# AzureLeon1/DiffSpectra

Measured on AMD Instinct MI355X. Metric: molecules/sec, 1000-step QM9S all-spectra sampling (partial run), higher is better.
Workload: dtype f32 (GEMMs as split-fp16 x3 MFMA with fp32 accumulate; fp32-level accuracy, parity gates unchanged)

## Files before the change

diffspectra_amd/csrc/ds_forward.hip:

```cpp
#include <hip/hip_runtime.h>
#include <math.h>
#include <stdint.h>
#include <stdlib.h>

#include <atomic>
#include <mutex>
#include <utility>
#include <vector>

#include "../../include/diffspectra_hip.h"
#include "../../include/diffspectra_step.h"
#include "../../include/diffspectra_tiles.h"
#include "ds_device.h"
#include "ds_host.h"

#define ADAC DS_ADA_COLS
constexpr int DS_NODE_PF = 8;
constexpr int DS_NODE_PF2 = 4;
constexpr int DS_QKV_PF = 4;
constexpr int DS_QKV_PF_WIDE = 4;
constexpr int DS_NODE_TILE64_MIN_PER_CU = 4;
constexpr int DS_TWO_STREAM_MAX_PAIRS = 400000;

#ifdef DS_STAMPS
// ... 787 lines not shown
#pragma unroll
        for (int cc = 0; cc < 2; ++cc) {
          const float bf = b1[half * 256 + (wave + 4 * cc) * 32 + (tid & 31)];
#pragma unroll
          for (int i = 0; i < 16; ++i) acc[cc][0][i] = bf;
          acc_zero<1>(lo[cc]);
        }
        wave_mma_h_ring_t2<1, false, 16, DS_NODE_PF2>(&H2[0][0], 256, wstream_h(W1, 512, 256, (half * 8 + wave) * 32),
                                                     wstream_h(W1, 512, 256, (half * 8 + wave + 4) * 32), 0, acc[0], lo[0], acc[1], lo[1]);
#pragma unroll
        for (int cc = 0; cc < 2; ++cc) {
          split_finish<1>(acc[cc], lo[cc]);
          const int colf = (wave + 4 * cc) * 32 + (tid & 31);
#pragma unroll
          for (int i = 0; i < 16; i += 2) {
            f32x2 v;
            v.x = acc[cc][0][i]; v.y = acc[cc][0][i + 1];
            v = ds_silu2(v);
            const int r0 = acc_row(i, hhf);
            split_store1(&B1[r0][0], 256, colf, v.x);
            split_store1(&B1[r0 + 1][0], 256, colf, v.y);
          }
        }
      }
      __syncthreads();
      asm volatile("" ::: "memory");
      wave_mma_h_ring_t2<1, false, 16, DS_NODE_PF2>(&B1[0][0], 256, wstream_h(W2, 256, 512, wave * 32), wstream_h(W2, 256, 512, (wave + 4) * 32),
                                                   half * 16, acc2[0], lo2[0], acc2[1], lo2[1], half * 16);
      __syncthreads();
    }
    split_finish<1>(acc2[0], lo2[0]);
    split_finish<1>(acc2[1], lo2[1]);
    const int hhl = (tid & 63) >> 5;
    const bool two = mB - mA <= 1;
    bool isB[16];
#pragma unroll
    for (int i = 0; i < 16; ++i) isB[i] = rmol[acc_row(i, hhl)] != mA;
    const int rows_here = Nn - row0;
#pragma unroll
    for (int cc = 0; cc < 2; ++cc) {
      const int col = (wave + 4 * cc) * 32 + (tid & 31);
      const float gA = gAv[cc], gB = gBv[cc], bb = bbv[cc];
      const RowStore st = row_store<256>(c.ws.h + (size_t)row0 * 256 + (wave + 4 * cc) * 32);
#pragma unroll
      for (int i = 0; i < 16; ++i) {
        const int row = acc_row(i, hhl);
        float g = isB[i] ? gB : gA;
        if (!two) { const int m = rmol[row]; if (m != mA && m != mB) g = gsec[(size_t)m * ADAC + col]; }
        const float out = split_load1(&H2[row][0], 256, col) + g * (acc2[cc][0][i] + bb);
        split_store1(&H2[row][0], 256, col, out);
        if (row < rows_here) row_put(st, ((i & 3) + 8 * (i >> 2)) * 256 * 4, out);
      }
    }
  }
  __syncthreads();
  {
    const float* br = BW(c, blk, DS_BW_NODE_RO_B);
    auto ws_of = [&](int it) {
      return it < 2 ? wstream_h(BW(c, blk, DS_BW_NODE_RO_H), 64, 256, it * 32) : wstream_h(BW(c, blk, DS_BW_AC_H), 512, 256, (it - 2) * 32);
    };
    auto bias_of = [&](int it) { return it < 2 ? br[it * 32 + (tid & 31)] : 0.0f; };
    auto store_of = [&](int it, const f32x16 (&acc)[1]) {
      if (it < 2) acc_store<1, 768>(acc, c.ws.atom_hids + (size_t)row0 * 768 + 256 + 64 * blk + it * 32, Nn - row0, [](int, float v) { return v; });
      else acc_store<1, 512>(acc, c.ws.ac + (size_t)row0 * 512 + (it - 2) * 32, Nn - row0, [](int, float v) { return v; });
    };
#pragma unroll
    for (int pr = 0; pr < 2; ++pr) {
      asm volatile("" ::: "memory");
      const int itA = wave + 8 * pr, itB = itA + 4;
      f32x16 acc[2][1], lo[2][1];
      const float bA = bias_of(itA), bB = bias_of(itB);
#pragma unroll
      for (int i = 0; i < 16; ++i) { acc[0][0][i] = bA; acc[1][0][i] = bB; }
      acc_zero<1>(lo[0]); acc_zero<1>(lo[1]);
      wave_mma_h_ring_t2<1, false, 16, DS_NODE_PF2>(&H2[0][0], 256, ws_of(itA), ws_of(itB), 0, acc[0], lo[0], acc[1], lo[1]);
      split_finish<1>(acc[0], lo[0]);
      store_of(itA, acc[0]);
      split_finish<1>(acc[1], lo[1]);
      store_of(itB, acc[1]);
    }
    if (wave < 2) {
      asm volatile("" ::: "memory");
      const int it = 16 + wave;
      f32x16 acc[1], lo[1];
      acc_zero<1>(acc);
      acc_zero<1>(lo);
      wave_mma_h_ring<1, false, 16, DS_NODE_PF>(&H2[0][0], 256, BW(c, blk, DS_BW_AC_H), 512, 256, (it - 2) * 32, 0, acc, lo);
      split_finish<1>(acc, lo);
      store_of(it, acc);
    }
  }
}

constexpr int DS_GATE_SLOTS = 16;
template <bool N2E>
__global__ __launch_bounds__(512) void k_node_update64(Ctx c, int blk) {
  ds_fp16_saturate();
  constexpr int T = 64, LDH = 2 * 256 + 8, GS = DS_GATE_SLOTS;
  __shared__ __attribute__((aligned(16))) _Float16 B1[T][LDH];
  __shared__ __attribute__((aligned(16))) _Float16 H2[T][LDH];
  __shared__ __attribute__((aligned(16))) float G[GS][256];
  __shared__ int rmol[T], rslot[T], smol[T], nslot;
  const int tid = threadIdx.x, wave = tid >> 6, row0 = blockIdx.x * T;
  const int Nn = c.L.Nn;
  const float* ada = c.ws.ada;
  const float* gsec = ada + blk * DS_ADA_BLOCK_STRIDE + DS_ADA_NODE + 1280;
  float4 va[2][4], vh[2][4];
#pragma unroll
  for (int ps = 0; ps < 2; ++ps) {
    const size_t gr = (size_t)min(row0 + 8 * wave + 4 * ps + ((tid & 63) >> 4), Nn - 1);
    const float4* ap = reinterpret_cast<const float4*>(c.ws.attn + gr * 256) + (tid & 15);
    const float4* hp = reinterpret_cast<const float4*>(c.ws.h + gr * 256) + (tid & 15);
#pragma unroll
    for (int u = 0; u < 4; ++u) {
      va[ps][u] = ap[16 * u];
      vh[ps][u] = hp[16 * u];
    }
  }
  if (tid < T) {
    const bool in = row0 + tid < Nn;
    const int m = in ? c.L.node_mol[row0 + tid] : 0;
    const bool first = in && (tid == 0 || c.L.node_mol[row0 + tid - 1] != m);
    const unsigned long long starts = __ballot(first);
    const int slot = __popcll(starts & ((2ull << tid) - 1ull)) - 1;
    rmol[tid] = m;
    rslot[tid] = slot;
    if (first) smol[slot] = m;
    if (tid == 0) nslot = __popcll(starts);
  }
  __syncthreads();
  const int ns = nslot;
  {
    const int lane = tid & 63, g = lane >> 4, j = lane & 15;
    float4 vg[2][4], sh[2][4], sc[2][4], gv[2];
#pragma unroll
    for (int ps = 0; ps < 2; ++ps) {
      const int row = 8 * wave + 4 * ps + g;
      const float4* ad = reinterpret_cast<const float4*>(ada + (size_t)rmol[row] * ADAC + blk * DS_ADA_BLOCK_STRIDE + DS_ADA_NODE) + j;
#pragma unroll
      for (int u = 0; u < 4; ++u) {
        vg[ps][u] = ad[128 + 16 * u];
        sh[ps][u] = ad[192 + 16 * u];
        sc[ps][u] = ad[256 + 16 * u];
      }
    }
#pragma unroll
    for (int u = 0; u < 2; ++u)
      gv[u] = reinterpret_cast<const float4*>(gsec + (size_t)smol[min(wave + 8 * u, ns - 1)] * ADAC)[lane];
#pragma unroll
    for (int ps = 0; ps < 2; ++ps) {
      const int row = 8 * wave + 4 * ps + g;
      float4 r[4];
#pragma unroll
      for (int u = 0; u < 4; ++u) {
        if (row0 + row >= Nn) va[ps][u] = vh[ps][u] = make_float4(0, 0, 0, 0);
        if (N2E) split_store4(&B1[row][0], 256, 64 * u + 4 * j, va[ps][u]);
        r[u].x = vh[ps][u].x + vg[ps][u].x * va[ps][u].x; r[u].y = vh[ps][u].y + vg[ps][u].y * va[ps][u].y;
        r[u].z = vh[ps][u].z + vg[ps][u].z * va[ps][u].z; r[u].w = vh[ps][u].w + vg[ps][u].w * va[ps][u].w;
      }
      ln_mod_quad256(r, sh[ps], sc[ps]);
#pragma unroll
      for (int u = 0; u < 4; ++u) split_store4(&H2[row][0], 256, 64 * u + 4 * j, r[u]);
    }
#pragma unroll
    for (int u = 0; u < 2; ++u) reinterpret_cast<float4*>(&G[wave + 8 * u][0])[lane] = gv[u];
  }
  const float* W1 = BW(c, blk, DS_BW_FF1_H);
  const float* W2 = BW(c, blk, DS_BW_FF2_H);
  auto tail_ws = [&](int it) {
    return it < 2 ? wstream_h(BW(c, blk, DS_BW_NODE_RO_H), 64, 256, it * 32) : wstream_h(BW(c, blk, DS_BW_AC_H), 512, 256, (it - 2) * 32);
  };
  WRingH<DS_NODE_PF> ring, ring_n2e;
  const bool n2e = N2E && wave < 4 && row0 + (wave >> 1) * 32 < Nn;
  const WStreamH wsn = wstream_h(BW(c, blk, DS_BW_N2E_H), 64, 256, (wave & 1) * 32);
  if (n2e) wring_h<DS_NODE_PF>(ring_n2e, wsn, 0);
  wring_h<DS_NODE_PF>(ring, wstream_h(W1, 512, 256, wave * 32), 0);
  __syncthreads();
  if (N2E) {
    {
      const int mt = wave >> 1, cc = wave & 1;
      if (n2e) {
        f32x16 acc[1], lo[1];
        acc_zero<1>(acc);
        acc_zero<1>(lo);
        wave_mma_h_deep<1, false, 16, DS_NODE_PF>(&B1[mt * 32][0], 256, wsn, ring_n2e, 0, acc, lo);
        split_finish<1>(acc, lo);
        acc_store<1, 64>(acc, c.ws.u + (size_t)(row0 + mt * 32) * 64 + cc * 32, Nn - row0 - mt * 32, [](int, float v) { return v; });
      }
    }
    __syncthreads();
  }
  {
    const float* b1 = BW(c, blk, DS_BW_FF1_B);
    const WStreamH ws2 = wstream_h(W2, 256, 512, wave * 32);
    f32x16 acc2[2], lo2[2];
    acc_zero<2>(acc2);
    acc_zero<2>(lo2);
    const int col = wave * 32 + (tid & 31);
    const float bb = BW(c, blk, DS_BW_FF2_B)[col];
    for (int half = 0; half < 2; ++half) {
      {
        asm volatile("" ::: "memory");
        const int hhf = (tid & 63) >> 5;
        f32x16 acc[2], lo[2];
        const float bf = b1[half * 256 + col];
#pragma unroll
        for (int m = 0; m < 2; ++m)
#pragma unroll
          for (int i = 0; i < 16; ++i) acc[m][i] = bf;
        acc_zero<2>(lo);
        wave_mma_h_deep<2, false, 16, DS_NODE_PF>(&H2[0][0], 256, wstream_h(W1, 512, 256, (half * 8 + wave) * 32), ring, 0, acc, lo);
        wring_h<DS_NODE_PF>(ring, ws2, half * 16);
        split_finish<2>(acc, lo);
#pragma unroll
        for (int m = 0; m < 2; ++m)
#pragma unroll
          for (int i = 0; i < 16; i += 2) {
            f32x2 v;
            v.x = acc[m][i]; v.y = acc[m][i + 1];
            v = ds_silu2(v);
            const int r0 = m * 32 + acc_row(i, hhf);
            split_store1(&B1[r0][0], 256, col, v.x);
            split_store1(&B1[r0 + 1][0], 256, col, v.y);
          }
      }
      __syncthreads();
      asm volatile("" ::: "memory");
      wave_mma_h_deep<2, false, 16, DS_NODE_PF>(&B1[0][0], 256, ws2, ring, half * 16, acc2, lo2, half * 16);
      wring_h<DS_NODE_PF>(ring, half == 0 ? wstream_h(W1, 512, 256, (8 + wave) * 32) : tail_ws(wave), 0);
      __syncthreads();
    }
    split_finish<2>(acc2, lo2);
    float* Gx = reinterpret_cast<float*>(&B1[0][0]);
    if (ns > GS) {
      for (int idx = tid; idx < (ns - GS) * 64; idx += 512)
        reinterpret_cast<float4*>(Gx)[idx] = reinterpret_cast<const float4*>(gsec + (size_t)smol[GS + (idx >> 6)] * ADAC)[idx & 63];
      __syncthreads();
    }
    const int hhl = (tid & 63) >> 5;
    const int rows_here = Nn - row0;
    const RowStore st = row_store<256>(c.ws.h + (size_t)row0 * 256 + wave * 32);
#pragma unroll
    for (int m = 0; m < 2; ++m)
#pragma unroll
      for (int i = 0; i < 16; ++i) {
        const int row = m * 32 + acc_row(i, hhl), s = rslot[row];
        const float g = s < GS ? G[s][col] : Gx[(s - GS) * 256 + col];
        const float out = split_load1(&H2[row][0], 256, col) + g * (acc2[m][i] + bb);
        split_store1(&H2[row][0], 256, col, out);
        if (row < rows_here) row_put(st, (m * 32 + (i & 3) + 8 * (i >> 2)) * 256 * 4, out);
      }
  }
  __syncthreads();
  {
    const float* br = BW(c, blk, DS_BW_NODE_RO_B);
    const int mt = (wave >> 1) & 1, itl = 16 + (wave & 1);
    const bool last = wave >= 4 && row0 + mt * 32 < Nn;
#pragma unroll
    for (int pr = 0; pr < 2; ++pr) {
      asm volatile("" ::: "memory");
      const int it = wave + 8 * pr;
      const float bi = it < 2 ? br[it * 32 + (tid & 31)] : 0.0f;
      f32x16 acc[2], lo[2];
#pragma unroll
      for (int m = 0; m < 2; ++m)
#pragma unroll
        for (int i = 0; i < 16; ++i) acc[m][i] = bi;
      acc_zero<2>(lo);
      wave_mma_h_deep<2, false, 16, DS_NODE_PF>(&H2[0][0], 256, tail_ws(it), ring, 0, acc, lo);
      if (pr == 0) wring_h<DS_NODE_PF>(ring, tail_ws(wave + 8), 0);
      else if (last) wring_h<DS_NODE_PF>(ring, tail_ws(itl), 0);
      split_finish<2>(acc, lo);
      if (it < 2) acc_store<2, 768>(acc, c.ws.atom_hids + (size_t)row0 * 768 + 256 + 64 * blk + it * 32, Nn - row0, [](int, float v) { return v; });
      else acc_store<2, 512>(acc, c.ws.ac + (size_t)row0 * 512 + (it - 2) * 32, Nn - row0, [](int, float v) { return v; });
    }
    if (last) {
      asm volatile("" ::: "memory");
      f32x16 acc[1], lo[1];
      acc_zero<1>(acc);
      acc_zero<1>(lo);
      wave_mma_h_deep<1, false, 16, DS_NODE_PF>(&H2[mt * 32][0], 256, tail_ws(itl), ring, 0, acc, lo);
      split_finish<1>(acc, lo);
      acc_store<1, 512>(acc, c.ws.ac + (size_t)(row0 + mt * 32) * 512 + (itl - 2) * 32, Nn - row0 - mt * 32, [](int, float v) { return v; });
    }
  }
}

__global__ __launch_bounds__(256, 2) void k_edge_update(Ctx c, int blk) {
  ds_fp16_saturate();
  DS_STAMP_INIT();
  constexpr int R = 32, LDW = 64 + DS_LDP;
  __shared__ __attribute__((aligned(16))) float E2s[4][R][LDW];
  __shared__ __attribute__((aligned(16))) float Ds[4][R][LDW];
  __shared__ int idx_s[4][3][R];
  const int tid = threadIdx.x, wave = tid >> 6, lane = tid & 63, hh = lane >> 5, r31 = lane & 31;
  constexpr int LDW2 = 2 * 64 + 8;
  float(*E2)[LDW] = E2s[wave];
  _Float16* E2h = reinterpret_cast<_Float16*>(&E2s[wave][0][0]);
  _Float16* Dh = reinterpret_cast<_Float16*>(&Ds[wave][0][0]);
  int* rmol = idx_s[wave][0];
  int* rpa = idx_s[wave][1];
  int* rpb = idx_s[wave][2];
  const int Pp = c.L.Pp;
  const int row0 = (blockIdx.x * 4 + wave) * R;
  if (row0 >= Pp) return;
  const int valid = min(R, Pp - row0);
  const float* ada = c.ws.ada + blk * DS_ADA_BLOCK_STRIDE + DS_ADA_EDGE;
  if (lane < R) {
    const int p = min(row0 + lane, Pp - 1);
    rmol[lane] = c.L.pair_mol[p]; rpa[lane] = c.L.pair_a[p]; rpb[lane] = c.L.pair_b[p];
  }
  DS_STAMP(0);
  {
    const float4* bn = reinterpret_cast<const float4*>(BW(c, blk, DS_BW_N2E_B));
    float rm[4], rs[4], ra[4];
#pragma unroll
    for (int t = 0; t < 4; ++t) {
      const int k = 4 * (lane & 15) + t;
      rm[t] = k ? BW(c, blk, DS_BW_RBF_MEAN)[k - 1] : 0.0f;
      rs[t] = __builtin_amdgcn_rcpf(k ? BW(c, blk, DS_BW_RBF_STD)[k - 1] : 1.0f);
      ra[t] = __builtin_amdgcn_rcpf(k ? BW(c, blk, DS_BW_RBF_ASTD)[k - 1] : 1.0f);
    }
#pragma unroll
    for (int it = 0; it < 2; ++it) {
      float4 ua[4], ub[4], ve[4], vd[4], vg[4], sh[4], sc[4];
      float xd[4];
#pragma unroll
      for (int u = 0; u < 4; ++u) {
        const int idx = lane + (it * 4 + u) * 64, row = idx >> 4, k4 = idx & 15;
        const size_t pc = (size_t)min(row0 + row, Pp - 1);
        const float* ad = ada + (size_t)rmol[row] * ADAC;
        ua[u] = reinterpret_cast<const float4*>(c.ws.u + (size_t)rpa[row] * 64)[k4];
        ub[u] = reinterpret_cast<const float4*>(c.ws.u + (size_t)rpb[row] * 64)[k4];
        ve[u] = reinterpret_cast<const float4*>(c.ws.e + pc * 64)[k4];
        xd[u] = c.ws.dist[pc];
        vg[u] = reinterpret_cast<const float4*>(ad + 128)[k4];
        sh[u] = reinterpret_cast<const float4*>(ad + 192)[k4];
        sc[u] = reinterpret_cast<const float4*>(ad + 256)[k4];
      }
#pragma unroll
      for (int u = 0; u < 4; ++u) {
        const int idx = lane + (it * 4 + u) * 64, row = idx >> 4, k4 = idx & 15;
        const float4 b = bn[k4];
        float4 r;
        r.x = ve[u].x + vg[u].x * ((ua[u].x + ub[u].x) + b.x); r.y = ve[u].y + vg[u].y * ((ua[u].y + ub[u].y) + b.y);
        r.z = ve[u].z + vg[u].z * ((ua[u].z + ub[u].z) + b.z); r.w = ve[u].w + vg[u].w * ((ua[u].w + ub[u].w) + b.w);
        r = ln_mod_reg64(r, sh[u], sc[u]);
        {
          float f[4];
#pragma unroll
          for (int t = 0; t < 4; ++t) {
            const float z = (xd[u] - rm[t]) * rs[t];
            f[t] = __expf(-0.5f * (z * z)) * ra[t];
          }
          if (k4 == 0) f[0] = xd[u];
          vd[u] = make_float4(f[0], f[1], f[2], f[3]);
        }
        if (row >= valid) { r = make_float4(0, 0, 0, 0); vd[u] = r; }
        split_store4(E2h + row * LDW2, 64, 4 * k4, r);
        split_store4(Dh + row * LDW2, 64, 4 * k4, vd[u]);
      }
    }
  }
  DS_STAMP(1);
  f32x16 a4[2][1], a4lo[2][1];
  acc_zero<1>(a4[0]); acc_zero<1>(a4[1]);
  acc_zero<1>(a4lo[0]); acc_zero<1>(a4lo[1]);
  {
    const float* b3 = BW(c, blk, DS_BW_FF3_B);
    const float* W3 = BW(c, blk, DS_BW_FF3_H);
    const uint4* W4 = reinterpret_cast<const uint4*>(BW(c, blk, DS_BW_FF4_C)) + lane;
#pragma unroll
    for (int hc = 0; hc < 4; ++hc) {
      f32x16 a3[1], a3lo[1];
#pragma unroll
      for (int q = 0; q < 4; ++q) {
        const float4 bb = *reinterpret_cast<const float4*>(b3 + hc * 32 + 8 * q + 4 * hh);
        a3[0][4 * q] = bb.x; a3[0][4 * q + 1] = bb.y; a3[0][4 * q + 2] = bb.z; a3[0][4 * q + 3] = bb.w;
      }
      acc_zero<1>(a3lo);
      wave_mma_h<1, true, 4>(E2h, 64, W3, 128, 64, hc * 32, 0, 4, a3, a3lo);
      split_finish<1>(a3, a3lo);
#pragma unroll
      for (int s_ = 0; s_ < 2; ++s_) {
        h8 y1, y2;
#pragma unroll
        for (int j = 0; j < 8; j += 2) {
          f32x2 v;
          v.x = a3[0][8 * s_ + j]; v.y = a3[0][8 * s_ + j + 1];
          v = ds_silu2(v);
          y1[j] = (_Float16)v.x; y1[j + 1] = (_Float16)v.y;
          y2[j] = (_Float16)((v.x - (float)y1[j]) * 2048.0f); y2[j + 1] = (_Float16)((v.y - (float)y1[j + 1]) * 2048.0f);
        }
#pragma unroll
        for (int ft = 0; ft < 2; ++ft) {
          const h8 w1 = __builtin_bit_cast(h8, W4[(((0 * 4 + hc) * 2 + s_) * 2 + ft) * 64]);
          const h8 w2 = __builtin_bit_cast(h8, W4[(((1 * 4 + hc) * 2 + s_) * 2 + ft) * 64]);
          a4[ft][0] = __builtin_amdgcn_mfma_f32_32x32x16_f16(w1, y1, a4[ft][0], 0, 0, 0);
          a4lo[ft][0] = __builtin_amdgcn_mfma_f32_32x32x16_f16(w1, y2, a4lo[ft][0], 0, 0, 0);
          a4lo[ft][0] = __builtin_amdgcn_mfma_f32_32x32x16_f16(w2, y1, a4lo[ft][0], 0, 0, 0);
        }
      }
    }
    split_finish<1>(a4[0], a4lo[0]);
    split_finish<1>(a4[1], a4lo[1]);
  }
  DS_STAMP(2);
  {
    const float* b4 = BW(c, blk, DS_BW_FF4_B);
    const float* grow = ada + (size_t)rmol[r31] * ADAC + 320;
    float4 xo[2][4];
#pragma unroll
    for (int ft = 0; ft < 2; ++ft)
#pragma unroll
      for (int q = 0; q < 4; ++q) {
        const int n0 = ft * 32 + 8 * q + 4 * hh;
        const float4 g = *reinterpret_cast<const float4*>(grow + n0);
        const float4 bb = *reinterpret_cast<const float4*>(b4 + n0);
        const h4 p0 = *reinterpret_cast<const h4*>(E2h + r31 * LDW2 + n0);
        const h4 p1 = *reinterpret_cast<const h4*>(E2h + r31 * LDW2 + 64 + n0);
        float4 x;
        x.x = fmaf((float)p1[0], 1.0f / 2048.0f, (float)p0[0]); x.y = fmaf((float)p1[1], 1.0f / 2048.0f, (float)p0[1]);
        x.z = fmaf((float)p1[2], 1.0f / 2048.0f, (float)p0[2]); x.w = fmaf((float)p1[3], 1.0f / 2048.0f, (float)p0[3]);
        x.x += g.x * (a4[ft][0][4 * q + 0] + bb.x); x.y += g.y * (a4[ft][0][4 * q + 1] + bb.y);
        x.z += g.z * (a4[ft][0][4 * q + 2] + bb.z); x.w += g.w * (a4[ft][0][4 * q + 3] + bb.w);
        xo[ft][q] = x;
      }
    __builtin_amdgcn_fence(__ATOMIC_ACQ_REL, "workgroup");
    __builtin_amdgcn_wave_barrier();
#pragma unroll
    for (int ft = 0; ft < 2; ++ft)
#pragma unroll
      for (int q = 0; q < 4; ++q) *reinterpret_cast<float4*>(&E2[r31][ft * 32 + 8 * q + 4 * hh]) = xo[ft][q];
  }
#pragma unroll
  for (int u = 0; u < 8; ++u) {
    const int idx = lane + u * 64, row = idx >> 4, k4 = idx & 15;
    const float4 v = reinterpret_cast<const float4*>(&E2[row][0])[k4];
    if (row < valid) reinterpret_cast<float4*>(c.ws.e + (size_t)(row0 + row) * 64)[k4] = v;
  }
  DS_STAMP(3);
  {
    f32x16 acc[1];
    acc_zero<1>(acc);
    wave_mma<1>(&E2[0][0], LDW, BW(c, blk, DS_BW_EDGE_RO_W), 32, 0, 0, 8, acc);
    if (r31 < 16) {
      const float b = BW(c, blk, DS_BW_EDGE_RO_B)[r31];
      acc_store<1, 192>(acc, c.ws.edge_hids + (size_t)row0 * 192 + 64 + 16 * blk, valid, [b](int, float v) { return v + b; });
    }
  }
  DS_STAMP(4);
  {
    float4 v[8];
#pragma unroll
    for (int u = 0; u < 8; ++u) v[u] = reinterpret_cast<const float4*>(&E2[(lane + u * 64) >> 4][0])[lane & 15];
    __builtin_amdgcn_fence(__ATOMIC_ACQ_REL, "workgroup");
    __builtin_amdgcn_wave_barrier();
#pragma unroll
    for (int u = 0; u < 8; ++u) split_store4(E2h + ((lane + u * 64) >> 4) * LDW2, 64, 4 * (lane & 15), v[u]);
  }
  DS_STAMP(5);
  {
    const float* bd = BW(c, blk, DS_BW_ED_B);
    const float* Wd = BW(c, blk, DS_BW_ED_H);
    float* ed = c.ws.ed + (size_t)row0 * 256;
    for (int ch = 0; ch < 8; ++ch) {
      asm volatile("" ::: "memory");
      f32x16 acc[1], lo[1];
      const float b = bd[ch * 32 + r31];
#pragma unroll
      for (int i = 0; i < 16; ++i) acc[0][i] = b;
      acc_zero<1>(lo);
      wave_mma_h<1>(E2h, 64, Wd, 256, 128, ch * 32, 0, 4, acc, lo);
      wave_mma_h<1>(Dh, 64, Wd, 256, 128, ch * 32, 4, 8, acc, lo, 4);
      split_finish<1>(acc, lo);
      acc_store<1, 256>(acc, ed + ch * 32, valid, [](int, float v) { return v; });
    }
  }
  DS_STAMP(6);
  DS_STAMP_FLUSH(0);
}

constexpr int EQUI_NCW = 4;
constexpr int EQUI_NLW = 4;
__global__ __launch_bounds__((EQUI_NCW + EQUI_NLW) * 64) void k_equi_pairs(Ctx c, int blk) {
  ds_fp16_saturate();
  constexpr int NCW = EQUI_NCW, NLW = EQUI_NLW;
  constexpr int T = 64, TP = 32, LDH = 2 * 256 + 8, NCH = 8;
  constexpr int CPW = NCH / NCW;
  constexpr int PPW = TP / NLW;
  constexpr int NPASS = PPW / 2;
  static_assert(NCH % NCW == 0 && TP % NLW == 0 && PPW % 2 == 0, "role split");
  static_assert(CPW == 2, "a consumer wave runs its two feature chunks against shared X fragments");
  __shared__ __attribute__((aligned(16))) _Float16 Xh[2][T][LDH];
  __shared__ __attribute__((aligned(16))) float part[2][NCH][T][4];
  __shared__ __attribute__((aligned(16))) float dirs[3][T][4];
  __shared__ __attribute__((aligned(16))) float cb0[NCH][2][16];
  __shared__ __attribute__((aligned(16))) float cw2[NCH][2][4][16];
  const int tid = threadIdx.x, wave = tid >> 6, lane = tid & 63, hh = lane >> 5;
  const int Pp = c.L.Pp;
  const int ntiles_all = (Pp + TP - 1) / TP;
  const int tiles_per_wg = (ntiles_all + (int)gridDim.x - 1) / (int)gridDim.x;
  const int ntiles = min(ntiles_all, ((int)blockIdx.x + 1) * tiles_per_wg);
  const float* adq = c.ws.ada + blk * DS_ADA_BLOCK_STRIDE + DS_ADA_EQUI;
  const bool consumer = wave < NCW;
  const float cscale = BW(c, blk, DS_BW_COORD_SCALE)[0];
  DS_STAMP_INIT();
  {
    const float* b0 = BW(c, blk, DS_BW_CM0_B);
    const float* w2 = BW(c, blk, DS_BW_CM2_W);
    for (int idx = tid; idx < NCH * 2 * 16; idx += (NCW + NLW) * 64) {
      const int ch = idx >> 5, h = (idx >> 4) & 1, i = idx & 15, f = ch * 32 + acc_row(i, h);
      cb0[ch][h][i] = b0[f];
#pragma unroll
      for (int o = 0; o < 3; ++o) cw2[ch][h][o][i] = wp_at(w2, 32, f, o);
      cw2[ch][h][3][i] = 0.0f;
    }
  }
  if (consumer) __builtin_amdgcn_s_setprio(0); else __builtin_amdgcn_s_setprio(3);

  const int lw = __builtin_amdgcn_readfirstlane(wave - NCW);

  auto tail = [&](int tile, int pb, int gen) {
    const int p0 = tile * TP;
    const int npairs = min(TP, Pp - p0);
    if ((lane >> 1) < npairs) {
      float4 sacc = reinterpret_cast<const float4*>(&part[pb][0][lane][0])[0];
#pragma unroll
      for (int w = 1; w < NCH; ++w) {
        const float4 pw = reinterpret_cast<const float4*>(&part[pb][w][lane][0])[0];
        sacc.x += pw.x; sacc.y += pw.y; sacc.z += pw.z;
      }
      const float inv[3] = {ds_tanh(sacc.x), ds_tanh(sacc.y), ds_tanh(sacc.z)};
      const float4 d = reinterpret_cast<const float4*>(&dirs[gen][lane][0])[0];
      const int bits = __float_as_int(d.w);
      const float w = ((inv[0] + ((bits & 1) ? inv[1] : 0.0f)) + ((bits & 2) ? inv[2] : 0.0f)) * (1.0f / 3.0f);
      float4 t;
      t.x = d.x * w; t.y = d.y * w; t.z = d.z * w; t.w = 0.0f;
      reinterpret_cast<float4*>(c.ws.tr)[(size_t)p0 * 2 + lane] = t;
    }
  };

  const int first = blockIdx.x * tiles_per_wg, stride = 1;
  if (first >= ntiles) return;
  if (consumer) {
    constexpr int PF = 4;
    WStreamH wsh[CPW];
#pragma unroll
    for (int cc = 0; cc < CPW; ++cc) wsh[cc] = wstream_h(BW(c, blk, DS_BW_CM0_H), 256, 256, (wave + NCW * cc) * 32);
    WRingH<PF> ring;
    wring_h<PF>(ring, wsh[0], 0);
    WRingH<PF> ringB;
    wring_h<PF>(ringB, wsh[1], 0);
    __syncthreads();
    DS_STAMP(0);
    int it = 0;
    for (int tile = first; tile < ntiles; tile += stride, ++it) {
      const int buf = it & 1;
      auto bias_init = [&](int ch, f32x16 (&acc1)[2]) {
        const float4* bp = reinterpret_cast<const float4*>(&cb0[ch][hh][0]);
#pragma unroll
        for (int m = 0; m < 2; ++m)
#pragma unroll
          for (int q4 = 0; q4 < 4; ++q4) {
            const float4 bv = bp[q4];
            acc1[m][4 * q4] = bv.x; acc1[m][4 * q4 + 1] = bv.y; acc1[m][4 * q4 + 2] = bv.z; acc1[m][4 * q4 + 3] = bv.w;
          }
      };
      auto epilogue = [&](int ch, const f32x16 (&acc1)[2]) {
        f32x2 so[2][3];
#pragma unroll
        for (int m = 0; m < 2; ++m)
#pragma unroll
          for (int o = 0; o < 3; ++o) so[m][o] = f32x2{0.0f, 0.0f};
#pragma unroll
        for (int q4 = 0; q4 < 4; ++q4) {
          float4 wv[3];
#pragma unroll
          for (int o = 0; o < 3; ++o) wv[o] = reinterpret_cast<const float4*>(&cw2[ch][hh][o][0])[q4];
#pragma unroll
          for (int m = 0; m < 2; ++m) {
            f32x2 y0, y1;
            y0.x = acc1[m][4 * q4]; y0.y = acc1[m][4 * q4 + 1]; y1.x = acc1[m][4 * q4 + 2]; y1.y = acc1[m][4 * q4 + 3];
            y0 = ds_silu2(y0); y1 = ds_silu2(y1);
#pragma unroll
            for (int o = 0; o < 3; ++o) {
              so[m][o] = __builtin_elementwise_fma(f32x2{wv[o].x, wv[o].y}, y0, so[m][o]);
              so[m][o] = __builtin_elementwise_fma(f32x2{wv[o].z, wv[o].w}, y1, so[m][o]);
            }
          }
        }
        float4 o4;
        float* op = &o4.x;
#pragma unroll
        for (int o = 0; o < 3; ++o) {
          const float s0 = so[0][o].x + so[0][o].y, s1 = so[1][o].x + so[1][o].y;
          const auto sw = __builtin_amdgcn_permlane32_swap(__float_as_uint(s0), __float_as_uint(s1), false, false);
          op[o] = __uint_as_float(sw[0]) + __uint_as_float(sw[1]);
        }
        o4.w = 0.0f;
        reinterpret_cast<float4*>(&part[buf][ch][lane][0])[0] = o4;
      };
      {
        f32x16 accA[2], loA[2], accB[2], loB[2];
        bias_init(wave, accA);
        bias_init(wave + NCW, accB);
        acc_zero<2>(loA);
        acc_zero<2>(loB);
        wave_mma_h_deep_t2<2, true, 16, PF>(&Xh[buf][0][0], 256, wsh[0], wsh[1], ring, ringB, 0, accA, loA, accB, loB);
        wring_h<PF>(ring, wsh[0], 0);
        wring_h<PF>(ringB, wsh[1], 0);
        DS_STAMP(3);
        split_finish<2>(accA, loA);
        epilogue(wave, accA);
        DS_STAMP(10);
        split_finish<2>(accB, loB);
        epilogue(wave + NCW, accB);
        DS_STAMP(11);
      }
      if (wave == 0 && it > 0) tail(tile - stride, buf ^ 1, (it + 2) % 3);
      DS_STAMP(1);
      __syncthreads();
      DS_STAMP(2);
    }
    if (wave == 0) tail(ntiles - 1, (it + 1) & 1, (it + 2) % 3);
    DS_STAMP_FLUSH(0);
  } else {
    const int g = lane >> 4, j = lane & 15, up = g >> 1, gdir = g & 1, slot = (lane >> 1) & (PPW - 1), dir = lane & 1;
    const float4* ac4 = reinterpret_cast<const float4*>(c.ws.ac);
    const float4* ed4 = reinterpret_cast<const float4*>(c.ws.ed);
    int pv_c = 0, av_c = 0, bv_c = 0, mv_c = 0, adj_c = 0;
    int pv_x = 0, av_x = 0, bv_x = 0, mv_x = 0, adj_x = 0;
#define DS_EQUI_FETCH_IDX(TILE, PV, AV, BV, MV, ADJ)                                                   \
    do {                                                                                               \
      const int p0_ = (TILE) * TP, qv_ = lw * PPW + slot;                                              \
      PV = qv_ < min(TP, Pp - p0_) ? p0_ + qv_ : 0;  \
      AV = c.L.pair_a[PV]; BV = c.L.pair_b[PV]; MV = c.L.pair_mol[PV]; ADJ = c.ws.adj[PV];             \
    } while (0)
#define DS_EQUI_ISSUE_B(BT, BVREG)                                                                     \
    do {                                                                                               \
      const int r0_ = __builtin_amdgcn_readlane(BVREG, 4 * (BT)), r1_ = __builtin_amdgcn_readlane(BVREG, 4 * (BT) + 2); \
      const float4* pb_ = ac4 + (size_t)(up ? r1_ : r0_) * 128 + (gdir ? 0 : 64) + j;                  \
      _Pragma("unroll") for (int u = 0; u < 4; ++u) Bv[BT][u] = pb_[16 * u];                           \
    } while (0)
    float4 Bv[NPASS][4], Ka[4], sh[4], sc[4];
    int cur_m = -1, cur_a = -1;
    DS_EQUI_FETCH_IDX(first, pv_c, av_c, bv_c, mv_c, adj_c);
    float4 pr = make_float4(0, 0, 0, 0), pc = pr;
    if (lane < 2 * PPW) {
      pr = reinterpret_cast<const float4*>(c.ws.pos)[dir ? bv_c : av_c];
      pc = reinterpret_cast<const float4*>(c.ws.pos)[dir ? av_c : bv_c];
    }
    if (first + stride < ntiles) DS_EQUI_FETCH_IDX(first + stride, pv_x, av_x, bv_x, mv_x, adj_x);
#pragma unroll
    for (int bt = 0; bt < NPASS; ++bt) DS_EQUI_ISSUE_B(bt, bv_c);
    DS_STAMP(4);
    int k = 0;
    for (int tile = first;; tile += stride, ++k) {
      const bool have = tile < ntiles;
      if (have) {
        const int buf = k & 1, gen = k % 3;
        const int p0 = tile * TP, npairs = min(TP, Pp - p0);
        const bool have_next = tile + stride < ntiles;
        int na[PPW], pm[PPW], pp[PPW];
#pragma unroll
        for (int u = 0; u < PPW; ++u) {
          pp[u] = __builtin_amdgcn_readlane(pv_c, 2 * u); na[u] = __builtin_amdgcn_readlane(av_c, 2 * u);
          pm[u] = __builtin_amdgcn_readlane(mv_c, 2 * u);
        }
#define DS_EQUI_ISSUE_A(BT)                                                                            \
        do {                                                                                           \
          const int ra_ = up ? na[2 * (BT) + 1] : na[2 * (BT)];                                        \
          if (ra_ != cur_a) {                                                                          \
            const float4* pa_ = ac4 + (size_t)ra_ * 128 + (gdir ? 64 : 0) + j;                         \
            _Pragma("unroll") for (int u = 0; u < 4; ++u) Ka[u] = pa_[16 * u];                         \
            cur_a = ra_;                                                                               \
          }                                                                                            \
        } while (0)
#define DS_EQUI_ISSUE_M(BT)                                                                            \
        do {                                                                                           \
          const int m_ = up ? pm[2 * (BT) + 1] : pm[2 * (BT)];                                         \
          if (m_ != cur_m) {                                                                           \
            const float4* ps_ = reinterpret_cast<const float4*>(adq + (size_t)m_ * ADAC) + j;          \
            _Pragma("unroll") for (int u = 0; u < 4; ++u) { sh[u] = ps_[16 * u]; sc[u] = ps_[64 + 16 * u]; }  \
            cur_m = m_;                                                                                \
          }                                                                                            \
        } while (0)
        DS_EQUI_ISSUE_A(0);
        DS_EQUI_ISSUE_M(0);
#pragma unroll
        for (int i = 0; i < PPW; ++i)
          __builtin_amdgcn_global_load_lds((const __attribute__((address_space(1))) void*)(ed4 + (size_t)pp[i] * 64 + lane),
                                           (__attribute__((address_space(3))) void*)&Xh[buf][2 * (lw * PPW + i)][0], 16, 0, 0);
        __builtin_amdgcn_sched_barrier(0);
        DS_STAMP(5);
        if (lane < 2 * PPW) {
          const float dx = pr.x - pc.x, dy = pr.y - pc.y, dz = pr.z - pc.z;
          const float nrm = fmaxf(__builtin_amdgcn_sqrtf(dx * dx + dy * dy + dz * dz), 1e-8f);
          const float sn = cscale * __builtin_amdgcn_rcpf(nrm);
          float4 d;
          d.x = dx * sn; d.y = dy * sn; d.z = dz * sn; d.w = __int_as_float(adj_c);
          reinterpret_cast<float4*>(&dirs[gen][2 * (lw * PPW + slot) + dir][0])[0] = d;
          if (have_next) {
            pr = reinterpret_cast<const float4*>(c.ws.pos)[dir ? bv_x : av_x];
            pc = reinterpret_cast<const float4*>(c.ws.pos)[dir ? av_x : bv_x];
          }
        }
        DS_STAMP(6);
        asm volatile("s_waitcnt vmcnt(0)" ::: "memory");
        __builtin_amdgcn_sched_barrier(0);
        DS_STAMP(8);
#pragma unroll
        for (int bt = 0; bt < NPASS; ++bt) {
          const int q = lw * PPW + 2 * bt + up;
          float4 x[4];
#pragma unroll
          for (int u = 0; u < 4; ++u) {
            const float4 e = reinterpret_cast<const float4*>(&Xh[buf][2 * q][0])[16 * u + j];
            x[u].x = (Ka[u].x + Bv[bt][u].x) + e.x; x[u].y = (Ka[u].y + Bv[bt][u].y) + e.y;
            x[u].z = (Ka[u].z + Bv[bt][u].z) + e.z; x[u].w = (Ka[u].w + Bv[bt][u].w) + e.w;
          }
          __builtin_amdgcn_sched_barrier(0);
          if (have_next) DS_EQUI_ISSUE_B(bt, bv_x);
          if (bt + 1 < NPASS) DS_EQUI_ISSUE_A(bt + 1);
          __builtin_amdgcn_sched_barrier(0);
          DS_STAMP(12);
          ln_mod_quad256(x, sh, sc);
          _Float16* xr = &Xh[buf][2 * q + gdir][0];
#pragma unroll
          for (int u = 0; u < 4; ++u) split_store4(xr, 256, 64 * u + 4 * j, x[u]);
          if (bt + 1 < NPASS) DS_EQUI_ISSUE_M(bt + 1);
          DS_STAMP(14);
        }
        if (npairs < TP) {
          for (int i = 0; i < PPW; ++i) {
            const int qz = lw * PPW + i;
            if (qz >= npairs) {
              float4* z = reinterpret_cast<float4*>(&Xh[buf][2 * qz][0]);
              z[lane] = make_float4(0, 0, 0, 0);
              z[64 + lane] = make_float4(0, 0, 0, 0);
              if (lane < 2) z[128 + lane] = make_float4(0, 0, 0, 0);
            }
          }
        }
      }
      DS_STAMP(7);
      __syncthreads();
      DS_STAMP(9);
      if (!have) break;
      pv_c = pv_x; av_c = av_x; bv_c = bv_x; mv_c = mv_x; adj_c = adj_x;
      if (tile + 2 * stride < ntiles) DS_EQUI_FETCH_IDX(tile + 2 * stride, pv_x, av_x, bv_x, mv_x, adj_x);
    }
#undef DS_EQUI_FETCH_IDX
#undef DS_EQUI_ISSUE_B
#undef DS_EQUI_ISSUE_A
#undef DS_EQUI_ISSUE_M
    DS_STAMP_FLUSH(NCW * 64);
  }
}

__global__ __launch_bounds__(64) void k_pos_update(Ctx c, int last) {
  const int m = blockIdx.x, r = threadIdx.x;
  const int n0 = c.L.node_off[m], n = c.L.node_off[m + 1] - n0;
  const int p0 = c.L.pair_off[m];
  if (n <= 0) return;
  float x = 0.0f, y = 0.0f, z = 0.0f;
  if (r < n) {
    const float4* tr = reinterpret_cast<const float4*>(c.ws.tr);
    float sx = 0.0f, sy = 0.0f, sz = 0.0f;
    for (int c0 = 0; c0 < n; c0 += 8) {
      float4 t[8];
#pragma unroll
      for (int u = 0; u < 8; ++u) {
        const int cc = c0 + u;
        t[u] = make_float4(0, 0, 0, 0);
        if (cc < n && cc != r) {
          const int lo = r < cc ? r : cc, hi = r < cc ? cc : r;
          const int pl = lo * (2 * n - lo - 1) / 2 + (hi - lo - 1);
          t[u] = tr[(size_t)(p0 + pl) * 2 + (r < cc ? 0 : 1)];
        }
      }
#pragma unroll
// ... 508 lines not shown
```

Measured before the change: 238.7.

## Share edge-decoder GEMM across waves so each weight chunk is loaded once per block

The final edge-decoder GEMM is restructured so that, after a workgroup barrier, each wave computes two of the eight 32-column output chunks for all 128 rows of the block. Before, every wave ran all eight chunks for only its own 32 rows. Each weight fragment is now fetched once per workgroup instead of four times, and the loads go through a register prefetch ring that overlaps them with the MFMAs. The cost is higher register pressure from 4x accumulators plus the ring, and a new __syncthreads. Waves with no valid rows can no longer return early, so they must still take part in the shared compute.

Result: faster. 243.8 (median of 6 runs) (+2.1%).

```diff
diff --git a/diffspectra_amd/csrc/ds_forward.hip b/diffspectra_amd/csrc/ds_forward.hip
--- a/diffspectra_amd/csrc/ds_forward.hip
+++ b/diffspectra_amd/csrc/ds_forward.hip
@@ -1113,9 +1113,8 @@
   int* rpa = idx_s[wave][1];
   int* rpb = idx_s[wave][2];
   const int Pp = c.L.Pp;
-  const int row0 = (blockIdx.x * 4 + wave) * R;
-  if (row0 >= Pp) return;
-  const int valid = min(R, Pp - row0);
+  const int wg_row0 = blockIdx.x * 4 * R, row0 = wg_row0 + wave * R;
+  const int valid = max(0, min(R, Pp - row0));
   const float* ada = c.ws.ada + blk * DS_ADA_BLOCK_STRIDE + DS_ADA_EDGE;
   if (lane < R) {
     const int p = min(row0 + lane, Pp - 1);
@@ -1261,6 +1260,11 @@
     }
   }
   DS_STAMP(4);
+  constexpr int ED_PF = 4;
+  const float* Wd = BW(c, blk, DS_BW_ED_H);
+  const WStreamH wsd[2] = {wstream_h(Wd, 256, 128, (2 * wave) * 32), wstream_h(Wd, 256, 128, (2 * wave + 1) * 32)};
+  WRingH<ED_PF> ring;
+  wring_h<ED_PF>(ring, wsd[0], 0);
   {
     float4 v[8];
 #pragma unroll
@@ -1271,24 +1275,52 @@
     for (int u = 0; u < 8; ++u) split_store4(E2h + ((lane + u * 64) >> 4) * LDW2, 64, 4 * (lane & 15), v[u]);
   }
   DS_STAMP(5);
+  __syncthreads();
+  DS_STAMP(6);
   {
     const float* bd = BW(c, blk, DS_BW_ED_B);
-    const float* Wd = BW(c, blk, DS_BW_ED_H);
-    float* ed = c.ws.ed + (size_t)row0 * 256;
-    for (int ch = 0; ch < 8; ++ch) {
-      asm volatile("" ::: "memory");
-      f32x16 acc[1], lo[1];
+    const _Float16* xe = reinterpret_cast<const _Float16*>(&E2s[0][0][0]) + r31 * LDW2 + 8 * hh;
+    const _Float16* xd = reinterpret_cast<const _Float16*>(&Ds[0][0][0]) + r31 * LDW2 + 8 * hh;
+    float* ed = c.ws.ed + (size_t)wg_row0 * 256;
+#pragma unroll
+    for (int c2 = 0; c2 < 2; ++c2) {
+      const int ch = 2 * wave + c2;
+      f32x16 acc[4], lo[4];
       const float b = bd[ch * 32 + r31];
 #pragma unroll
-      for (int i = 0; i < 16; ++i) acc[0][i] = b;
-      acc_zero<1>(lo);
-      wave_mma_h<1>(E2h, 64, Wd, 256, 128, ch * 32, 0, 4, acc, lo);
-      wave_mma_h<1>(Dh, 64, Wd, 256, 128, ch * 32, 4, 8, acc, lo, 4);
-      split_finish<1>(acc, lo);
-      acc_store<1, 256>(acc, ed + ch * 32, valid, [](int, float v) { return v; });
-    }
-  }
-  DS_STAMP(6);
+      for (int m = 0; m < 4; ++m)
+#pragma unroll
+        for (int i = 0; i < 16; ++i) acc[m][i] = b;
+      acc_zero<4>(lo);
+#pragma unroll
+      for (int i = 0; i < 8; ++i) {
+        __builtin_amdgcn_sched_barrier(0);
+        const _Float16* xr = (i < 4 ? xe : xd) + (i & 3) * 16;
+        h8 x1[4], x2[4];
+#pragma unroll
+        for (int m = 0; m < 4; ++m) {
+          x1[m] = *reinterpret_cast<const h8*>(xr + m * R * LDW2);
+          x2[m] = *reinterpret_cast<const h8*>(xr + m * R * LDW2 + 64);
+        }
+        const h8 w1 = ring.w1[i % ED_PF], w2 = ring.w2[i % ED_PF];
+#pragma unroll
+        for (int m = 0; m < 4; ++m) lo[m] = __builtin_amdgcn_mfma_f32_32x32x16_f16(x2[m], w1, lo[m], 0, 0, 0);
+#pragma unroll
+        for (int m = 0; m < 4; ++m) acc[m] = __builtin_amdgcn_mfma_f32_32x32x16_f16(x1[m], w1, acc[m], 0, 0, 0);
+#pragma unroll
+        for (int m = 0; m < 4; ++m) lo[m] = __builtin_amdgcn_mfma_f32_32x32x16_f16(x1[m], w2, lo[m], 0, 0, 0);
+        if (i + ED_PF < 8) {
+          ring.w1[i % ED_PF] = wload_h(wsd[c2], 0, i + ED_PF); ring.w2[i % ED_PF] = wload_h(wsd[c2], 1, i + ED_PF);
+        } else if (c2 == 0) {
+          ring.w1[i % ED_PF] = wload_h(wsd[1], 0, i + ED_PF - 8); ring.w2[i % ED_PF] = wload_h(wsd[1], 1, i + ED_PF - 8);
+        }
+        __builtin_amdgcn_sched_barrier(0);
+      }
+      split_finish<4>(acc, lo);
+      acc_store<4, 256>(acc, ed + ch * 32, Pp - wg_row0, [](int, float v) { return v; });
+    }
+  }
+  DS_STAMP(7);
   DS_STAMP_FLUSH(0);
 }
 
```
